# dtarb/TauDEM

Measured on NVIDIA H100. Metric: Mcells/s for aread8+areadinf on synthetic fractal DEM, higher is better.
Workload: dtype f32

## Files before the change

taudem_b200/csrc/sweep_warp.cu:

```cuda
#include <stddef.h>
#include <string.h>

#include <algorithm>

#include "ctx.h"
#include "dinf_common.cuh"
#include "kernels.h"
#include "rowfact.cuh"

namespace td {
namespace {

constexpr int TS = 32;
constexpr int TH = 32;
constexpr int RS = TS + 4;
constexpr int RH = TH + 2;
constexpr int RN = RH * RS + 4;
#ifndef TD_WSTK
#define TD_WSTK 128
#endif
constexpr int STKCAP = TD_WSTK;
constexpr unsigned NODE_VALID = 0x8000u, NODE_CON = 0x1000u;
constexpr unsigned FULL = 0xffffffffu;
constexpr int EXP_NO_CARRY = 16;
#ifdef TD_EMU
constexpr int MAXSH = 8;
#else
constexpr int MAXSH = 64;
#endif
constexpr int C_TERM = 3 * MAXSH * 16, C_ACTIVE = (3 * MAXSH + 1) * 16, C_WORDS = (3 * MAXSH + 2) * 16;

constexpr unsigned pack_dir(bool row) {
  unsigned v = 0;
  for (int k = 1; k <= 8; ++k) v |= (unsigned)((row ? drow(k) : dcol(k)) + 1) << (2 * k);
  return v;
}
constexpr unsigned DROW_LUT = pack_dir(true), DCOL_LUT = pack_dir(false);
__device__ __forceinline__ int lut_drow(int k) { return (int)((DROW_LUT >> (2 * k)) & 3u) - 1; }
__device__ __forceinline__ int lut_dcol(int k) { return (int)((DCOL_LUT >> (2 * k)) & 3u) - 1; }

template <bool DINF>
struct __align__(16) WarpMem {
  float area[RN];
  float ang[DINF ? RN : 4];
  unsigned short node[RN];
  alignas(16) unsigned cnt[TS * TH / 4];
  unsigned short stk[DINF ? STKCAP : 2];
  unsigned short ext[DINF ? 256 : 128];
  unsigned evmask[TH];
  int sp, next, ovf, pad;
};
template <bool DINF> constexpr int workers_per_cta() { return DINF ? 16 : 26; }
static_assert(sizeof(WarpMem<false>) * workers_per_cta<false>() <= 227 * 1024 && sizeof(WarpMem<true>) * workers_per_cta<true>() + 1024 <= 227 * 1024,
              "the workers of a CTA must fit the shared memory of an SM");
static_assert(offsetof(WarpMem<true>, ang) % 16 == 0 && offsetof(WarpMem<true>, node) % 8 == 0 && offsetof(WarpMem<false>, node) % 8 == 0, "cp.async alignment");

struct PeerStrip {
  unsigned* cntw = nullptr; int* state = nullptr; int* tq = nullptr; unsigned long long* ctr = nullptr; float* halo_in = nullptr;
  unsigned qmask = 0; int ntx = 0, ny = 0, valid = 0, nsh = 1, qshift = 0;
};

struct WArgs {
  const unsigned short* node;
  unsigned* cntw;
  float* area;
  const float* w;
  const float* ang;
  Strip s;
  int usew, contcheck;
  float w_nodata;
  const double* theta;
  const double* dxc;
  int* halo;
  int ntx, nty, th;
  const float* dm; float dm_nodata;
  const float* dist;
  SweepExtra x;
  int* state;
  int* tq;
  unsigned qmask;
  int nsh, qshift;
  PropRow prop;
  double dx0;
  unsigned long long* ctr;
  unsigned long long* stat;
  int stats, exp;
  int peer;
  PeerStrip up, down;
  unsigned long long* G;
  const float* halo_in;
};

#ifdef TD_EMU
template <typename T> __device__ __forceinline__ T ldv(const T* p) { emu::yield(); return *((const volatile T*)p); }
#else
template <typename T> __device__ __forceinline__ T ldv(const T* p) { return *((const volatile T*)p); }
#endif
template <typename T> __device__ __forceinline__ void stv(T* p, T v) { *((volatile T*)p) = v; }

#ifndef TD_EMU
__device__ __forceinline__ void cp16(void* smem, const void* g) { asm volatile("cp.async.cg.shared.global [%0], [%1], 16;" ::"r"(smem_u32(smem)), "l"(g) : "memory"); }
__device__ __forceinline__ void cp8(void* smem, const void* g) { asm volatile("cp.async.ca.shared.global [%0], [%1], 8;" ::"r"(smem_u32(smem)), "l"(g) : "memory"); }
__device__ __forceinline__ void cp4(void* smem, const void* g) { asm volatile("cp.async.ca.shared.global [%0], [%1], 4;" ::"r"(smem_u32(smem)), "l"(g) : "memory"); }
__device__ __forceinline__ void cp_wait_all() { asm volatile("cp.async.wait_all;" ::: "memory"); }
#else
__device__ __forceinline__ void cp_check(const void* smem, const void* g, size_t n) { if ((size_t)smem % n || (size_t)g % n) { fprintf(stderr, "emu: misaligned %zu-byte cp.async\n", n); abort(); } }
__device__ __forceinline__ void cp16(void* smem, const void* g) { emu::yield(); cp_check(smem, g, 16); memcpy(smem, g, 16); }
__device__ __forceinline__ void cp8(void* smem, const void* g) { cp_check(smem, g, 8); memcpy(smem, g, 8); }
__device__ __forceinline__ void cp4(void* smem, const void* g) { cp_check(smem, g, 4); memcpy(smem, g, 4); }
__device__ __forceinline__ void cp_wait_all() {}
#endif

#define W_ADD(ptr, v) (a.peer ? atomicAdd_system((ptr), (v)) : atomicAdd((ptr), (v)))
#define W_CAS(ptr, c, v) (a.peer ? atomicCAS_system((ptr), (c), (v)) : atomicCAS((ptr), (c), (v)))
#define W_EXCH(ptr, v) (a.peer ? atomicExch_system((ptr), (v)) : atomicExch((ptr), (v)))
#define W_ADD_IF(sys, ptr, v) ((sys) ? atomicAdd_system((ptr), (v)) : atomicAdd((ptr), (v)))
#define W_CAS_IF(sys, ptr, c, v) ((sys) ? atomicCAS_system((ptr), (c), (v)) : atomicCAS((ptr), (c), (v)))
#define W_EXCH_IF(sys, ptr, v) ((sys) ? atomicExch_system((ptr), (v)) : atomicExch((ptr), (v)))

__device__ __forceinline__ unsigned long long* w_head(unsigned long long* ctr, int q) { return ctr + (3 * q) * 16; }
__device__ __forceinline__ unsigned long long* w_tail(unsigned long long* ctr, int q) { return ctr + (3 * q + 1) * 16; }
__device__ __forceinline__ unsigned long long* w_done(unsigned long long* ctr, int q) { return ctr + (3 * q + 2) * 16; }

__device__ void sched_push(const WArgs& a, int t) {
  const int q = t & (a.nsh - 1);
  const unsigned long long slot = W_ADD(w_tail(a.ctr, q), 1ull);
  int* ring = a.tq + ((size_t)q << a.qshift) + (slot & a.qmask);
  while (W_CAS(ring, 0, t + 1) != 0) {}
}
__device__ __forceinline__ bool edge_tile(const WArgs& a, int t) { return a.peer && (t < a.ntx || t >= (a.nty - 1) * a.ntx); }
__device__ void sched_activate(const WArgs& a, int t) {
  const bool sys = edge_tile(a, t);
  for (;;) {
    const int st = W_CAS_IF(sys, a.state + t, 0, 1);
    if (st == 0) { sched_push(a, t); return; }
    if (st == 1 || st == 3) return;
    if (W_CAS_IF(sys, a.state + t, 2, 3) == 2) return;
  }
}
__device__ void sched_activate_peer(const WArgs& a, const PeerStrip& P, int t) {
  for (;;) {
    const int st = atomicCAS_system(P.state + t, 0, 1);
    if (st == 0) {
      atomicAdd_system(a.G, 1ull);
      const int q = t & (P.nsh - 1);
      const unsigned long long slot = atomicAdd_system(w_tail(P.ctr, q), 1ull);
      int* ring = P.tq + ((size_t)q << P.qshift) + (slot & P.qmask);
      while (atomicCAS_system(ring, 0, t + 1) != 0) {}
      __threadfence_system();
      if (atomicExch_system(P.ctr + C_ACTIVE, 1ull) == 1ull) atomicAdd_system(a.G, ~0ull);
      return;
    }
    if (st == 1 || st == 3) return;
    if (atomicCAS_system(P.state + t, 2, 3) == 2) return;
  }
}
template <int ALG>
__device__ void deliver_peer(const WArgs& a, bool up, int c_src, float val, int c_dst) {
  const PeerStrip& P = up ? a.up : a.down;
  const int pitch = a.s.pitch;
  P.halo_in[(up ? pitch : 0) + c_src] = val;
  if (ALG == 9) P.halo_in[2 * pitch + (up ? pitch : 0) + c_src] = ldv(a.x.out3 + a.s.idx(up ? 1 : a.s.ny, c_src));
  __threadfence_system();
  const int r = up ? P.ny : 1;
  const long long ci = (long long)r * pitch + c_dst;
  const unsigned sh = (unsigned)(ci & 3) * 8u;
  const unsigned old = atomicAdd_system(P.cntw + (ci >> 2), 0u - (1u << sh));
  if (((old >> sh) & 0xffu) == 1u) sched_activate_peer(a, P, ((r - 1) / a.th) * P.ntx + c_dst / TS);
}
__device__ __forceinline__ int ld_relaxed(const int* p) {
#ifdef TD_EMU
  emu::yield(); return *((const volatile int*)p);
#else
  int v; asm volatile("ld.relaxed.gpu.global.s32 %0, [%1];" : "=r"(v) : "l"(p) : "memory"); return v;
#endif
}
__device__ __forceinline__ long long ld_relaxed(const unsigned long long* p) {
#ifdef TD_EMU
  emu::yield(); return (long long)*((const volatile unsigned long long*)p);
#else
  long long v; asm volatile("ld.relaxed.gpu.global.s64 %0, [%1];" : "=l"(v) : "l"(p) : "memory"); return v;
#endif
}
__device__ __forceinline__ void idle_wait(unsigned cycles) {
#ifdef TD_EMU
  (void)cycles; emu::yield();
#else
  const long long t0 = clock64();
  do { __nanosleep(cycles >> 1); } while (clock64() - t0 < (long long)cycles);
#endif
}
__device__ __forceinline__ void fence_acquire(bool sys) {
#ifdef TD_EMU
  (void)sys; emu::yield();
#else
  if (sys) asm volatile("fence.acquire.sys;" ::: "memory");
  else asm volatile("fence.acquire.gpu;" ::: "memory");
#endif
}
__device__ __forceinline__ void fence_release(bool sys) {
#ifdef TD_EMU
  (void)sys; emu::yield();
#else
  if (sys) asm volatile("fence.release.sys;" ::: "memory");
  else asm volatile("fence.release.gpu;" ::: "memory");
#endif
}
__device__ __forceinline__ uint4 ld_cnt4(const uint4* p, bool sys) {
#ifdef TD_EMU
  (void)sys; return __ldcg(p);
#else
  uint4 v;
  if (sys) asm volatile("ld.relaxed.sys.global.v4.u32 {%0,%1,%2,%3}, [%4];" : "=r"(v.x), "=r"(v.y), "=r"(v.z), "=r"(v.w) : "l"(p) : "memory");
  else asm volatile("ld.relaxed.gpu.global.v4.u32 {%0,%1,%2,%3}, [%4];" : "=r"(v.x), "=r"(v.y), "=r"(v.z), "=r"(v.w) : "l"(p) : "memory");
  return v;
#endif
}
__device__ bool sched_balanced(const WArgs& a) {
  long long d = 0, t = 0;
#pragma unroll 16
  for (int q = 0; q < a.nsh; ++q) d += ld_relaxed(w_done(a.ctr, q));
  fence_acquire(false);
#pragma unroll 16
  for (int q = 0; q < a.nsh; ++q) t += ld_relaxed(w_tail(a.ctr, q));
  return d == t;
}
__device__ int sched_pop(const WArgs& a, int q, bool scanner) {
  const unsigned long long h = atomicAdd(w_head(a.ctr, q), 1ull);
  int* slot = a.tq + ((size_t)q << a.qshift) + (h & a.qmask);
  unsigned wait = 512, n = 0;
  for (;;) {
    const int v = ld_relaxed(slot);
    if (v != 0) {
      W_EXCH(slot, 0);
      const int prev = W_EXCH_IF(edge_tile(a, v - 1), a.state + (v - 1), 2);
      return prev == 0x7ffffff0 ? -1 : v - 1;
    }
    if ((++n & 7u) == 0u) {
      if (ld_relaxed(a.ctr + C_TERM) != 0) return -1;
      if (scanner && (n & 63u) == 0u && sched_balanced(a)) {
        bool over = true;
        if (a.peer) {
          if (atomicExch_system(a.ctr + C_ACTIVE, 0ull) == 1ull) {
            __threadfence_system();
            if (sched_balanced(a)) atomicAdd_system(a.G, ~0ull);
            else if (atomicExch_system(a.ctr + C_ACTIVE, 1ull) == 1ull) atomicAdd_system(a.G, ~0ull);
          }
          over = ldv(a.G) == 0ull;
        }
        if (over) { atomicExch(a.ctr + C_TERM, 1ull); return -1; }
      }
    }
    idle_wait(wait);
    if (wait < 4096) wait <<= 1;
  }
}
__device__ __forceinline__ int sched_release(const WArgs& a, int t, bool dirty) {
  return dirty ? 3 : W_CAS_IF(edge_tile(a, t), a.state + t, 2, 0);
}
__device__ void sched_finish(const WArgs& a, int t, int rel, bool pay) {
  if (rel != 2) { W_EXCH_IF(edge_tile(a, t), a.state + t, 1); sched_push(a, t); }
  if (pay) atomicAdd(w_done(a.ctr, t & (a.nsh - 1)), 1ull);
}

__global__ void k_zero_words(unsigned* p, size_t n) {
  for (size_t i = (size_t)blockIdx.x * blockDim.x + threadIdx.x; i < n; i += (size_t)gridDim.x * blockDim.x) p[i] = 0u;
}
__global__ void k_fill_floats(float* p, size_t n, float v) {
  for (size_t i = (size_t)blockIdx.x * blockDim.x + threadIdx.x; i < n; i += (size_t)gridDim.x * blockDim.x) p[i] = v;
}
unsigned fill_grid(size_t n) {
  int dev = 0, sms = 0;
  if (cudaGetDevice(&dev) != cudaSuccess || cudaDeviceGetAttribute(&sms, cudaDevAttrMultiProcessorCount, dev) != cudaSuccess || sms < 1) sms = 1;
  return (unsigned)std::max<size_t>(1, std::min<size_t>((n + 255) / 256, (size_t)sms * 16));
}
}
cudaError_t fill_floats(float* p, const Strip& s, float v, cudaStream_t st) {
  const size_t n = (size_t)s.cells();
  const unsigned grid = fill_grid(n);
  k_fill_floats<<<grid, 256, 0, st>>>(p, n, v);
  TD_LAUNCHED();
  return cudaGetLastError();
}
cudaError_t zero_words(void* p, size_t bytes, cudaStream_t st) {
  const size_t n = bytes / 4;
  const unsigned grid = fill_grid(n);
  k_zero_words<<<grid, 256, 0, st>>>((unsigned*)p, n);
  TD_LAUNCHED();
  return cudaGetLastError();
}
namespace {
__global__ void k_wsched_init(int* state, int* tq, int ntiles, unsigned long long* ctr, unsigned long long* stat, int nsh, int qshift, unsigned qmask) {
  const unsigned i = blockIdx.x * blockDim.x + threadIdx.x;
  if ((int)i < ntiles) {
    state[i] = 1;
    const int q = (int)i & (nsh - 1);
    const unsigned long long slot = atomicAdd(w_tail(ctr, q), 1ull);
    tq[((size_t)q << qshift) + (slot & qmask)] = (int)i + 1;
  }
  if (i == 0) {
    ctr[C_ACTIVE] = 1ull;
    for (int j = 0; j < 9; ++j) stat[j] = 0;
  }
}

__device__ __noinline__ double wshare_full(float ang, double t, int kk) {
  const Outflow o = dinf_outflow(ang, t);
  return o.k1 == kk ? o.p1 : o.p2;
}
struct __align__(16) Sector { double lo, hi, den, rden; };

__device__ __forceinline__ unsigned zero_bytes(unsigned w) { return ~(((w & 0x7f7f7f7fu) + 0x7f7f7f7fu) | w) & 0x80808080u; }
__device__ __forceinline__ unsigned zero_nibble(unsigned w) {
  const unsigned z = zero_bytes(w);
  return ((z >> 7) & 1u) | ((z >> 14) & 2u) | ((z >> 21) & 4u) | ((z >> 28) & 8u);
}

template <int ALG, typename Mem>
__device__ __forceinline__ float gridnet_eval(const WArgs& a, const Mem& M, int ri, unsigned msk, int r, int c) {
  const Strip& s = a.s;
  if (a.dm && a.dm[s.idx(r, c)] == 0.f) return a.w_nodata;
  const float* drowp = a.dist + (size_t)(min(r, s.ny) - 1) * 8;
  float val = 0.f, a1 = 0.f, a2 = 0.f;
#pragma unroll
  for (int k = 1; k <= 8; ++k) {
    if (!(msk & (1u << (k - 1)))) continue;
    const int ni = ri + drow(k) * RS + dcol(k);
    if ((((unsigned)M.node[ni] >> 8) & 0xfu) == 0u) continue;
    if (a.dm && a.dm[s.idx(r + drow(k), c + dcol(k))] == 0.f) continue;
    const float an = M.area[ni];
    const float d = drowp[k - 1];
    if (ALG == 4) { const float ld = an + d; if (ld > val) val = ld; }
    else if (ALG == 5) val = val + (an + d);
    else { if (an >= a1) { a2 = a1; a1 = an; } else if (an > a2) a2 = an; }
  }
  if (ALG == 6) val = (a2 + 1.f > a1) ? a2 + 1.f : a1;
  return val;
}

struct Eval { float val; bool con; };
template <bool USEW, int ALG, typename Mem>
__device__ __forceinline__ Eval d8_gather(const WArgs& a, const Mem& M, int ri, unsigned msk, int r, int c, float wv, float NOD, bool con) {
  if (ALG >= 4) return {gridnet_eval<ALG>(a, M, ri, msk, r, c), con};
  if (USEW) {
    float val = (ALG == 0 && nd_f(wv, a.w_nodata)) ? -1.0f : wv;
#pragma unroll
    for (int k = 1; k <= 8; ++k)
      if (msk & (1u << (k - 1))) {
        const float an = M.area[ri + drow(k) * RS + dcol(k)];
        if (nd_f(an, NOD)) con = true;
        else val = ALG == 0 ? val + an : ALG == 1 ? (an > val ? an : val) : (an < val ? an : val);
      }
    return {val, con};
  }
  float val = 1.0f, mn = 0.f;
#pragma unroll
  for (int k = 1; k <= 8; ++k)
    if (msk & (1u << (k - 1))) {
      const float an = M.area[ri + drow(k) * RS + dcol(k)];
      val = val + an;
      mn = fminf(mn, an);
    }
  if (mn < 0.f) con = true;
  return {val, con};
}

__device__ __forceinline__ double dinf_share(const WArgs& a, const Sector* sect, unsigned f, float av, int kk, int rn) {
  if (a.prop.uniform && f != 9u) {
    const bool upper = f >= 10u;
    const int k1 = (int)(upper ? f - 8u : f);
    const bool first = kk == k1 && !upper;
    const bool wrap = k1 == 8 && !first && !upper;
    const Sector S = sect[wrap ? 0 : (upper ? k1 - 1 : k1)];
    double ad = (double)av;
    if (wrap) ad = (double)(float)(ad - 2.0 * TD_PI);
    const double num = first ? S.hi - ad : ad - S.lo;
    return a.prop.safe ? div_recip(num, S.den, S.rden) : num / S.den;
  }
  return wshare_full(av, a.prop.uniform ? a.prop.ar[2] : theta_of_row(a.theta, a.s.ny, min(max(rn, 0), a.s.ny + 1)), kk);
}

__device__ __forceinline__ double own_area(const WArgs& a, int r) { return a.prop.uniform ? a.dx0 : a.dxc[min(r, a.s.ny) - 1]; }

template <bool DINF, bool USEW, int ALG>
__global__ void __launch_bounds__(workers_per_cta<DINF>() * 32, 1) k_sweep_warp(const WArgs a) {
  extern __shared__ __align__(16) unsigned char dsm[];
  using Mem = WarpMem<DINF>;
  const Strip& s = a.s;
  const int lane = (int)(threadIdx.x & 31u), wid = (int)(threadIdx.x >> 5);
  const unsigned lt = (1u << lane) - 1u;
  Mem& M = *reinterpret_cast<Mem*>(dsm + (size_t)wid * sizeof(Mem));
  const int myq = (int)((blockIdx.x * (blockDim.x >> 5) + (unsigned)wid) & (unsigned)(a.nsh - 1));
  const float NOD = (ALG == 0 || (ALG >= 4 && ALG <= 6)) ? -1.0f : TD_MISSINGFLOAT;
  __shared__ Sector sect[9];
  if (DINF) {
    if (threadIdx.x < 9) { const int j = (int)threadIdx.x; sect[j].lo = a.prop.ar[j]; sect[j].hi = a.prop.ar[j + 1]; sect[j].den = a.prop.den[j]; sect[j].rden = a.prop.rden[j]; }
    __syncthreads();
  }

  int carry = -1;
  for (;;) {
    long long tk0 = 0, tk1 = 0, tk2 = 0, tk3 = 0;
    int t = carry;
    if (t < 0) {
      if (lane == 0) { if (a.stats) tk0 = clock64(); t = sched_pop(a, myq, wid == 0); if (a.stats) tk1 = clock64(); }
      t = __shfl_sync(FULL, t, 0);
      if (t < 0) return;
    } else if (a.stats && lane == 0) { tk0 = clock64(); tk1 = tk0; }
    carry = -1;
    const int ty = t / a.ntx, tx = t - ty * a.ntx;
    const int c0 = tx * TS, r0 = 1 + ty * TH;

    unsigned g0[8];
    {
      const int r = r0 + lane;
      uint4 qa = make_uint4(FULL, FULL, FULL, FULL), qb = qa;
      if (r <= s.ny) {
        const uint4* src = reinterpret_cast<const uint4*>(a.cntw + (s.idx(r, c0) >> 2));
        qa = ld_cnt4(src, a.peer); qb = ld_cnt4(src + 1, a.peer);
      }
      g0[0] = qa.x; g0[1] = qa.y; g0[2] = qa.z; g0[3] = qa.w; g0[4] = qb.x; g0[5] = qb.y; g0[6] = qb.z; g0[7] = qb.w;
      uint4* dst = reinterpret_cast<uint4*>(M.cnt + lane * 8);
      dst[0] = qa; dst[1] = qb;
      M.evmask[lane] = 0u;
    }
    if (lane == 0) { M.sp = 0; M.next = 0; M.ovf = 0; }
    fence_acquire(a.peer);
    __syncwarp();
#pragma unroll
    for (int j = 0; j < (RH * 8 + 31) / 32; ++j) {
      const int i = lane + 32 * j;
      if (i < RH * 8) {
        const int rr = i >> 3, q = i & 7;
        const int r = r0 - 1 + rr, c = c0 + 4 * q;
        const int so = rr * RS + 4 + 4 * q;
        if (r <= s.ny + 1) {
          const long long g = s.idx(r, c);
          if (a.peer && (r == 0 || r == s.ny + 1)) cp16(M.area + so, a.halo_in + (r == 0 ? 0 : s.pitch) + c);
          else cp16(M.area + so, a.area + g);
          if (DINF) cp16(M.ang + so, a.ang + g);
          cp8(M.node + so, a.node + g);
        } else {
          *reinterpret_cast<float4*>(M.area + so) = make_float4(NOD, NOD, NOD, NOD);
          if (DINF) *reinterpret_cast<float4*>(M.ang + so) = make_float4(0.f, 0.f, 0.f, 0.f);
          *reinterpret_cast<uint2*>(M.node + so) = make_uint2(0u, 0u);
        }
      }
    }
#pragma unroll
    for (int rr = lane; rr < RH; rr += 32) {
      const int r = r0 - 1 + rr;
      const bool rowok = r <= s.ny + 1;
      const bool halo_row = a.peer && (r == 0 || r == s.ny + 1);
      const float* hrow = a.halo_in + (r == 0 ? 0 : s.pitch);
      const int sw = rr * RS + 3, se = rr * RS + RS;
      const bool west = rowok && c0 > 0, east = rowok && c0 + TS < s.pitch;
      const long long gw_ = s.idx(r, c0 - 1), ge_ = s.idx(r, c0 + TS);
      float aw = NOD, ae = NOD;
      if (west) { aw = __ldcg(halo_row ? hrow + (c0 - 1) : a.area + gw_); if (DINF) cp4(M.ang + sw, a.ang + gw_); cp4(M.node + sw - 1, a.node + gw_ - 1); }
      else { M.node[sw - 1] = 0; M.node[sw] = 0; }
      if (east) { ae = __ldcg(halo_row ? hrow + (c0 + TS) : a.area + ge_); if (DINF) cp4(M.ang + se, a.ang + ge_); cp4(M.node + se, a.node + ge_); }
      else { M.node[se] = 0; M.node[se + 1] = 0; }
      M.area[sw] = aw; M.area[se] = ae;
    }
    unsigned rdy = 0;
#pragma unroll
    for (int j = 0; j < 8; ++j) rdy |= zero_nibble(g0[j]) << (4 * j);
    cp_wait_all();
    __syncwarp();
    if (a.stats && lane == 0) tk2 = clock64();

    int cur = -1;
    int iters = 0;
    for (;;) {
      if (cur < 0 && rdy) { const int b = __ffs(rdy) - 1; rdy &= rdy - 1; cur = lane * TS + b; }
      if (DINF) {
        const unsigned idle = __ballot_sync(FULL, cur < 0);
        if (idle) {
          const int n = min(ldv(&M.sp), STKCAP);
          if (n > 0) {
            const int take = min(__popc(idle), n);
            const int rank = __popc(idle & lt);
            if (cur < 0 && rank < take) cur = M.stk[n - 1 - rank];
            __syncwarp();
            if (lane == 0) M.sp = n - take;
          }
        }
      }
      const unsigned act = __ballot_sync(FULL, cur >= 0);
      if (ALG < 7 && act != 0u && (act & (act - 1u)) == 0u) {
        int c = __shfl_sync(FULL, cur, __ffs(act) - 1);
        bool forked = false;
        do {
          ++iters;
          const int lr = c >> 5, lx = c & 31;
          const int ri = (lr + 1) * RS + lx + 4;
          float wv = 0.f;
          if (USEW) wv = a.w[s.idx(r0 + lr, c0 + lx)];
          const unsigned nd = M.node[ri];
          const unsigned msk = nd & 0xffu;
          bool con = (nd & NODE_CON) != 0;
          float val;
          if (!DINF) { const Eval e = d8_gather<USEW, ALG>(a, M, ri, msk, r0 + lr, c0 + lx, wv, NOD, con); val = e.val; con = e.con; }
          else {
            double prod = 0.;
            if (lane < 8 && ((msk >> lane) & 1u)) {
              const int k = lane + 1;
              const int dr = lut_drow(k);
              const int ni = ri + dr * RS + lut_dcol(k);
              const unsigned f = ((unsigned)M.node[ni] >> 8) & 0xfu;
              const float av = M.ang[ni];
              const float an = M.area[ni];
              const double p = dinf_share(a, sect, f, av, k > 4 ? k - 4 : k + 4, r0 + lr + dr);
              if (ALG == 3) {
                const float dmv = __ldg(a.dm + s.idx(r0 + lr + dr, c0 + lx + lut_dcol(k)));
                prod = (nd_f(an, NOD) || nd_f(dmv, a.dm_nodata)) ? __longlong_as_double(0x7ff8dead00000000ll) : (double)(float)((double)(dmv * an) * p);
              } else prod = nd_f(an, NOD) ? __longlong_as_double(0x7ff8dead00000000ll) : p * (double)an;
            }
            val = 0.f;
            if (ALG == 3) val = USEW ? wv : (float)own_area(a, r0 + lr);
            for (unsigned m = msk; m; m &= m - 1u) {
              const double pr = __shfl_sync(FULL, prod, __ffs(m) - 1);
              if (pr != pr) con = true; else val = ALG == 3 ? val + (float)pr : (float)((double)val + pr);
            }
            if (ALG == 3) {}
            else if (USEW) val = val + wv;
            else val = (float)((double)val + own_area(a, r0 + lr));
          }
          if (con && a.contcheck) val = NOD;
          if (lane == 0) { M.area[ri] = val; M.evmask[lr] |= 1u << lx; }
          int next = -1;
#pragma unroll
          for (int j = 0; j < (DINF ? 2 : 1); ++j) {
            int k;
            if (!DINF) k = (int)((nd >> 8) & 0xfu);
            else k = j == 0 ? dinf_node_k1(nd) : dinf_node_k2(nd);
            if (k < 1 || k > 8) continue;
            const int nlr = lr + lut_drow(k), nlx = lx + lut_dcol(k);
            if ((unsigned)nlr < (unsigned)TH && (unsigned)nlx < (unsigned)TS && r0 + nlr <= s.ny) {
              const int l2 = nlr * TS + nlx;
              const unsigned sh = (unsigned)(l2 & 3) * 8u;
              unsigned w = 0;
              if (lane == 0) { w = M.cnt[l2 >> 2]; M.cnt[l2 >> 2] = w - (1u << sh); }
              w = __shfl_sync(FULL, w, 0);
              if (((w >> sh) & 0xffu) == 1u) {
                if (next < 0) next = l2;
                else {
                  forked = true;
                  if (lane == 0) { const int slot = M.sp; if (slot < STKCAP) M.stk[slot] = (unsigned short)l2; else if (a.stats) M.ovf = 1; M.sp = slot + 1; }
                }
              }
            } else if (s.on_grid(r0 + nlr, c0 + nlx)) {
              if (lane == 0) { M.ext[M.next] = (unsigned short)(c | ((k - 1) << 11)); M.next = M.next + 1; }
            }
          }
          c = next;
          __syncwarp();
        } while (c >= 0 && !forked);
        cur = lane == 0 ? c : -1;
        continue;
      }
      if (act == 0u) {
        if (!DINF) break;
        const unsigned ev = M.evmask[lane];
#pragma unroll
        for (int j = 0; j < 8; ++j) rdy |= zero_nibble(M.cnt[lane * 8 + j]) << (4 * j);
        rdy &= ~ev;
        if (__ballot_sync(FULL, rdy != 0u) == 0u) break;
        continue;
      }
      ++iters;
      if (cur >= 0) {
        const int l = cur;
        const int lr = l >> 5, lx = l & 31;
        const int ri = (lr + 1) * RS + lx + 4;
        float wv = 0.f;
        if (USEW) wv = a.w[s.idx(r0 + lr, c0 + lx)];
        const unsigned nd = M.node[ri];
        const unsigned msk = nd & 0xffu;
        bool con = (nd & NODE_CON) != 0;
        float val;
        int cont = -1;
        if (!DINF) { const Eval e = d8_gather<USEW, ALG>(a, M, ri, msk, r0 + lr, c0 + lx, wv, NOD, con); val = e.val; con = e.con; }
        else {
          const int r = r0 + lr;
          val = 0.f;
          float loadin = 0.f;
          if (ALG == 3) val = USEW ? wv : (float)own_area(a, r);
#pragma unroll 1
          for (unsigned m = msk; m; m &= m - 1u) {
            const int k = __ffs(m);
            const int dr = lut_drow(k);
            const int ni = ri + dr * RS + lut_dcol(k);
            const unsigned f = ((unsigned)M.node[ni] >> 8) & 0xfu;
            const float av = M.ang[ni];
            const float an = M.area[ni];
            const double p = dinf_share(a, sect, f, av, k > 4 ? k - 4 : k + 4, r + dr);
            if (ALG == 3) {
              const float dmv = __ldg(a.dm + s.idx(r + dr, c0 + lx + lut_dcol(k)));
              if (nd_f(an, NOD) || nd_f(dmv, a.dm_nodata)) con = true;
              else val = val + (float)((double)(dmv * an) * p);
            } else if (ALG == 7) {
              const long long gi = s.idx(r + dr, c0 + lx + lut_dcol(k));
              const float qq = __ldg(a.w + gi), dmm = __ldg(a.dm + gi);
              if (nd_f(an, NOD) || nd_f(dmm, a.dm_nodata) || nd_f(qq, a.w_nodata)) con = true;
              else val = (float)((double)val + ((p * (double)an) * (double)qq) * (double)dmm);
            } else if (ALG == 8 || ALG == 9) {
              float nt = 0.f;
              if (nd_f(an, NOD)) con = true; else { val = (float)((double)val + p * (double)an); nt = an; }
              if (ALG == 9) {
                const int rn = r + dr, cc = c0 + lx + lut_dcol(k);
                const float cn = (a.peer && (rn == 0 || rn == s.ny + 1)) ? ldv(a.halo_in + 2 * s.pitch + (rn == 0 ? 0 : s.pitch) + cc)
                                                                         : ldv(a.x.out3 + s.idx(rn, cc));
                if (nd_f(cn, NOD)) con = true; else loadin = (float)((double)loadin + (p * (double)nt) * (double)cn);
              }
            } else if (nd_f(an, NOD)) con = true; else val = (float)((double)val + p * (double)an);
          }
          if (ALG == 3) {}
          else if (ALG == 7) {
            const float dgv = (float)a.x.dg[s.idx(r, c0 + lx)];
            if (!(wv > 0.f)) { val = NOD; con = false; }
            else if (dgv > 0.f) { val = a.x.csol; con = false; }
            else val = val / wv;
          } else if (ALG == 8 || ALG == 9) {
            const long long gc = s.idx(r, c0 + lx);
            const float tcc = __ldg(a.dm + gc);
            float cinv = 0.f;
            bool ev = !nd_f(wv, a.w_nodata) && !nd_f(tcc, a.dm_nodata);
            if (ALG == 9) { cinv = __ldg(a.x.cin + gc); ev = ev && !nd_f(cinv, a.x.cin_nodata); }
            if (!ev) { val = NOD; con = false; }
            else {
              const float transin = val;
              float transout, depp;
              if ((transin + wv) > tcc) { transout = tcc; depp = transin + wv - transout; }
              else { transout = transin + wv; depp = 0.f; }
              float cs = 0.f;
              if (ALG == 9) {
                float loadout;
                if (transout < transin) loadout = transin > 0.f ? loadin * transout / transin : 0.f;
                else loadout = loadin + cinv * (transout - transin);
                cs = transout > 0.f ? loadout / transout : 0.f;
              }
              const bool bad = con && a.contcheck;
              a.x.out2[gc] = bad ? NOD : depp;
              if (ALG == 9) { stv(a.x.out3 + gc, bad ? NOD : cs); __threadfence_block(); }
              val = transout;
            }
          }
          else if (USEW) val = val + wv;
          else val = (float)((double)val + own_area(a, r));
        }
        if (con && a.contcheck) val = NOD;
        M.area[ri] = val;
        atomicOr(&M.evmask[lr], 1u << lx);
#pragma unroll
        for (int j = 0; j < (DINF ? 2 : 1); ++j) {
          int k;
          if (!DINF) k = (int)((nd >> 8) & 0xfu);
          else k = j == 0 ? dinf_node_k1(nd) : dinf_node_k2(nd);
          if (k < 1 || k > 8) continue;
          const int nlr = lr + lut_drow(k), nlx = lx + lut_dcol(k);
          if ((unsigned)nlr < (unsigned)TH && (unsigned)nlx < (unsigned)TS && r0 + nlr <= s.ny) {
            const int l2 = nlr * TS + nlx;
            const unsigned sh = (unsigned)(l2 & 3) * 8u;
            const unsigned old = atomicSub(&M.cnt[l2 >> 2], 1u << sh);
            if (((old >> sh) & 0xffu) == 1u) {
              if (cont < 0) cont = l2;
              else {
                const int slot = atomicAdd(&M.sp, 1);
                if (slot < STKCAP) M.stk[slot] = (unsigned short)l2; else if (a.stats) M.ovf = 1;
              }
            }
          } else if (s.on_grid(r0 + nlr, c0 + nlx)) {
            M.ext[atomicAdd(&M.next, 1)] = (unsigned short)(l | ((k - 1) << 11));
          }
        }
        cur = cont;
      }
      __syncwarp();
    }

    if (a.stats && lane == 0) tk3 = clock64();

    const unsigned evs = M.evmask[lane];
    for (unsigned rows = __ballot_sync(FULL, evs != 0u); rows; rows &= rows - 1u) {
      const int lr = __ffs(rows) - 1;
      const unsigned evr = __shfl_sync(FULL, evs, lr);
      if ((evr >> lane) & 1u) a.area[s.idx(r0 + lr, c0 + lane)] = M.area[(lr + 1) * RS + lane + 4];
    }
    unsigned dl[8];
    {
      const int myr = r0 + lane;
      const bool rimrow = lane == 0 || lane == TH - 1 || myr >= s.ny;
      unsigned* gw = a.cntw + (s.idx(min(myr, s.ny), c0) >> 2);
#pragma unroll
      for (int j = 0; j < 8; ++j) {
        const unsigned was = g0[j];
        unsigned now = M.cnt[lane * 8 + j];
        const unsigned keep = ((was >> 7) & 0x01010101u) * 0xffu;
        now = (now & ~keep) | (was & keep);
        const unsigned e4 = (evs >> (4 * j)) & 0xfu;
        dl[j] = now - was + ((e4 * 0x00204081u) & 0x01010101u) * 0xfeu;
        if (j >= 1 && j <= 6 && !rimrow && dl[j] != 0u) { gw[j] = was + dl[j]; dl[j] = 0u; }
      }
    }
    __syncwarp();
    fence_release(a.peer);
    const int ne = M.next;
    int pend = -1, pend_e = -1;
    auto cross = [&](int e, unsigned& old, unsigned& sh) -> int {
      const int l = M.ext[e] & 0x7ff, k = (M.ext[e] >> 11) + 1;
      const int lr = l >> 5, lx = l & 31;
      const int nlr = lr + lut_drow(k), nlx = lx + lut_dcol(k);
      const int r = r0 + nlr, c = c0 + nlx;
      if (r == 0 || r == s.ny + 1) {
        if (a.peer) deliver_peer<ALG>(a, r == 0, c0 + lx, M.area[(lr + 1) * RS + lx + 4], c);
        else atomicAdd(a.halo + (r == 0 ? 0 : s.pitch) + c, 1);
        return -1;
      }
      if (!((unsigned)M.node[(nlr + 1) * RS + nlx + 4] & NODE_VALID)) return -1;
      const long long ci = s.idx(r, c);
      sh = (unsigned)(ci & 3) * 8u;
      old = W_ADD_IF(a.peer && (r == 1 || r == s.ny), a.cntw + (ci >> 2), 0u - (1u << sh));
      return ((r - 1) / TH) * a.ntx + c / TS;
    };
    unsigned xo = 0u, xsh = 0u, ro[8];
    const int xt = lane < ne ? cross(lane, xo, xsh) : -1;
    const int myr = r0 + lane;
#pragma unroll
    for (int j = 0; j < 8; ++j) ro[j] = 0u;
    if (myr <= s.ny) {
      unsigned* gw = a.cntw + (s.idx(myr, c0) >> 2);
#pragma unroll
      for (int j = 0; j < 8; ++j)
        if (dl[j] != 0u) ro[j] = W_ADD_IF(a.peer && (myr == 1 || myr == s.ny), gw + j, dl[j]);
    }
    if (xt >= 0 && ((xo >> xsh) & 0xffu) == 1u) { pend = xt; pend_e = lane; }
    for (int e = lane + 32; e < ne; e += 32) {
      unsigned o, sh;
      const int tt = cross(e, o, sh);
      if (tt >= 0 && ((o >> sh) & 0xffu) == 1u) {
        if (pend >= 0) sched_activate(a, pend);
        pend = tt; pend_e = e;
      }
    }
    bool dirty = false;
#pragma unroll
    for (int j = 0; j < 8; ++j)
      if (dl[j] != 0u && zero_bytes(ro[j] + dl[j])) dirty = true;
    dirty = __ballot_sync(FULL, dirty) != 0u;
    int hi = pend_e;
#pragma unroll
    for (int d = 16; d >= 1; d >>= 1) hi = max(hi, __shfl_xor_sync(FULL, hi, d));
    const int wl = hi & 31;
    const int ct = hi >= 0 ? __shfl_sync(FULL, pend, wl) : -1;
    int claim = -1, rel = -1;
    if (hi >= 0 && lane == wl && !(a.exp & EXP_NO_CARRY)) claim = W_CAS_IF(edge_tile(a, ct), a.state + ct, 0, 2);
    if (lane == 0) rel = sched_release(a, t, dirty);
    if (hi >= 0) {
      if (lane == wl) {
        if (claim == 0) {
          carry = ct;
          if (a.stats) atomicAdd(a.stat, 1ull);
        } else sched_activate(a, ct);
      } else if (pend >= 0 && pend != ct) sched_activate(a, pend);
      carry = __shfl_sync(FULL, carry, wl);
    }
    __syncwarp();
    if (lane == 0) sched_finish(a, t, rel, carry < 0);
    if (a.stats) {
      int tot = __popc(evs);
#pragma unroll
      for (int d = 16; d >= 1; d >>= 1) tot += __shfl_xor_sync(FULL, tot, d);
      if (lane == 0) {
        const long long tk4 = clock64();
        atomicAdd(a.stat + 3, 1ull);
        atomicAdd(a.stat + 4, (unsigned long long)(tk1 - tk0));
        atomicAdd(a.stat + 5, (unsigned long long)(tk2 - tk1));
        atomicAdd(a.stat + 6, (unsigned long long)(tk3 - tk2));
        atomicAdd(a.stat + 7, (unsigned long long)(tk4 - tk3));
        atomicAdd(a.stat + 1, (unsigned long long)tot);
        atomicAdd(a.stat + 2, (unsigned long long)iters);
        if (DINF && M.ovf) atomicAdd(a.stat + 8, 1ull);
      }
    }
    __syncwarp();
  }
}

__global__ void k_wapply_halo(WArgs a, const int* __restrict__ dec_top, const int* __restrict__ dec_bot) {
  const int c = blockIdx.x * blockDim.x + threadIdx.x;
  if (c >= a.s.nx) return;
#pragma unroll
  for (int side = 0; side < 2; ++side) {
    const int* dec = side == 0 ? dec_top : dec_bot;
    if (dec == nullptr) continue;
    const int d = dec[c];
    if (d <= 0) continue;
    const int r = side == 0 ? 1 : a.s.ny;
    const long long ci = a.s.idx(r, c);
    if (!(a.node[ci] & NODE_VALID)) continue;
    const unsigned sh = (unsigned)(ci & 3) * 8u;
    const unsigned old = atomicAdd(a.cntw + (ci >> 2), 0u - ((unsigned)d << sh));
    if ((int)((old >> sh) & 0xffu) == d) sched_activate(a, ((r - 1) / a.th) * a.ntx + c / TS);
  }
}

__global__ void k_wsched_reset(unsigned long long* ctr) { for (int i = threadIdx.x; i < C_WORDS; i += blockDim.x) ctr[i] = (i == C_ACTIVE) ? 1ull : 0ull; }

int wargs(td_ctx* ctx, WArgs& a, const Strip& s) {
  a.s = s;
  a.area = nullptr; a.w = nullptr; a.ang = nullptr; a.dx0 = 0.; a.usew = 0; a.contcheck = 1; a.w_nodata = 0.f; a.theta = nullptr; a.dxc = nullptr; a.halo = nullptr; a.dm = nullptr; a.dm_nodata = 0.f; a.dist = nullptr;
  a.th = TH;
  a.ntx = (s.nx + TS - 1) / TS; a.nty = (s.ny + a.th - 1) / a.th;
  a.stats = 0; a.exp = 0;
  a.peer = 0; a.G = nullptr; a.halo_in = nullptr; a.up = PeerStrip(); a.down = PeerStrip();
  const long long nt = (long long)a.ntx * a.nty;
  if (nt > (1ll << 30)) { set_error("strip has too many tiles"); return TD_ERR_ARG; }
  int nsh = 1;
  while (nsh * 2 <= MAXSH && nsh * 2 <= nt) nsh *= 2;
  const unsigned long long need = (unsigned long long)((nt + nsh - 1) / nsh) + (1u << 13);
  int qshift = 14;
  while ((1ull << qshift) < need) ++qshift;
  a.nsh = nsh; a.qshift = qshift; a.qmask = (1u << qshift) - 1u;
  TD_CUDA(ctx->tileflags.ensure((size_t)nt * 4 + ((size_t)nsh << qshift) * 4));
  a.state = ctx->tileflags.as<int>();
  a.tq = a.state + nt;
  TD_CUDA(ctx->wsched.ensure(C_WORDS * sizeof(unsigned long long)));
  a.ctr = ctx->wsched.as<unsigned long long>();
  a.stat = ctx->d_ctr + 24;
  a.node = ctx->node.as<unsigned short>();
  a.cntw = ctx->cnt.as<unsigned>();
  return TD_OK;
}

enum : unsigned { NEED_W = 1, NEED_DM = 2, NEED_DIST = 4, NEED_EXTRA = 8, NEED_DG = 16, NEED_OUT2 = 32, NEED_CIN = 64, NEED_OUT3 = 128 };
using SweepLaunch = void (*)(const WArgs&, int, int, size_t, cudaStream_t);
template <bool D, bool U, int A>
void launch_sweep(const WArgs& a, int g, int threads, size_t smem, cudaStream_t st) {
  k_sweep_warp<D, U, A><<<g, threads, smem, st>>>(a);
}
struct SweepKernel {
  bool dinf, usew;
  int alg;
  unsigned need;
  const void* kern;
  SweepLaunch launch;
  int threads;
  size_t smem;
};
template <bool D, bool U, int A>
SweepKernel sweep_kernel(unsigned need) {
  return {D, U, A, need, (const void*)k_sweep_warp<D, U, A>, launch_sweep<D, U, A>, workers_per_cta<D>() * 32, sizeof(WarpMem<D>) * workers_per_cta<D>()};
}
const SweepKernel SWEEPS[] = {
    sweep_kernel<false, false, 0>(0), sweep_kernel<false, true, 0>(0), sweep_kernel<true, false, 0>(0), sweep_kernel<true, true, 0>(0),
    sweep_kernel<false, true, 1>(0), sweep_kernel<false, true, 2>(0),
    sweep_kernel<true, false, 3>(NEED_DM), sweep_kernel<true, true, 3>(NEED_DM),
    sweep_kernel<false, false, 4>(NEED_DIST), sweep_kernel<false, false, 5>(NEED_DIST), sweep_kernel<false, false, 6>(NEED_DIST),
    sweep_kernel<true, true, 7>(NEED_W | NEED_DM | NEED_EXTRA | NEED_DG),
    sweep_kernel<true, true, 8>(NEED_W | NEED_DM | NEED_EXTRA | NEED_OUT2),
    sweep_kernel<true, true, 9>(NEED_W | NEED_DM | NEED_EXTRA | NEED_OUT2 | NEED_CIN | NEED_OUT3),
};
static_assert(sizeof(SWEEPS) / sizeof(SWEEPS[0]) == td_ctx::SWEEP_KERNELS, "td_ctx::wgrid has one slot per sweep kernel");
}

int wsweep_begin(td_ctx* ctx, const Strip& s, cudaStream_t st) {
  WArgs a;
  if (int rc = wargs(ctx, a, s)) return rc;
  const int nt = a.ntx * a.nty;
  TD_CUDA(zero_words(a.ctr, C_WORDS * sizeof(unsigned long long), st));
  TD_CUDA(zero_words(a.tq, ((size_t)a.nsh << a.qshift) * sizeof(int), st));
  k_wsched_init<<<(nt + 255) / 256, 256, 0, st>>>(a.state, a.tq, nt, a.ctr, a.stat, a.nsh, a.qshift, a.qmask);
  TD_LAUNCHED();
  TD_CUDA(cudaGetLastError());
  return TD_OK;
}

int wsweep_apply_halo(td_ctx* ctx, const Strip& s, const int* dec_top, const int* dec_bot, cudaStream_t st) {
  WArgs a;
  if (int rc = wargs(ctx, a, s)) return rc;
  k_wsched_reset<<<1, 256, 0, st>>>(a.ctr);
  TD_LAUNCHED();
  k_wapply_halo<<<(s.nx + 255) / 256, 256, 0, st>>>(a, dec_top, dec_bot);
  TD_LAUNCHED();
  TD_CUDA(cudaGetLastError());
  return TD_OK;
}

int wsweep_run(td_ctx* ctx, bool dinf, float* area, const float* w, const float* ang, const Strip& s, float w_nodata, int usew,
               int contcheck, const double* theta, const double* dxc, int* halo, cudaStream_t st, int alg, const float* dm, float dm_nodata,
               const float* dist, const SweepExtra* extra) {
  int row = -1;
  for (int i = 0; i < td_ctx::SWEEP_KERNELS; ++i)
    if (SWEEPS[i].dinf == dinf && SWEEPS[i].usew == (usew != 0) && SWEEPS[i].alg == alg) row = i;
  const unsigned have = (w ? NEED_W : 0u) | (dm ? NEED_DM : 0u) | (dist ? NEED_DIST : 0u) |
                        (extra ? NEED_EXTRA | (extra->dg ? NEED_DG : 0u) | (extra->out2 ? NEED_OUT2 : 0u) | (extra->cin ? NEED_CIN : 0u) | (extra->out3 ? NEED_OUT3 : 0u) : 0u);
  if (row < 0) { set_error("wsweep_run: no sweep for this algebra with this flow model and weights"); return TD_ERR_ARG; }
  if (const unsigned miss = SWEEPS[row].need & ~have) {
    static const char* const grid[8] = {"w", "dm", "dist", "extra", "extra->dg", "extra->out2", "extra->cin", "extra->out3"};
    set_error(std::string("wsweep_run: algebra ") + std::to_string(alg) + " requires the grid " + grid[__builtin_ctz(miss)]);
    return TD_ERR_ARG;
  }
  const SweepKernel& K = SWEEPS[row];
  if (alg == 9 && ctx->peer_on && ctx->peer_halo.cap < sizeof(float) * 4 * (size_t)s.pitch) {
    set_error("wsweep_run: peer mode of the transport limited accumulation with a concentration needs the halo buffer of sweep_peer_export");
    return TD_ERR_ARG;
  }
  WArgs a;
  if (int rc = wargs(ctx, a, s)) return rc;
  a.area = area; a.w = w; a.ang = ang; a.usew = usew; a.contcheck = contcheck;
  a.w_nodata = w_nodata; a.theta = theta; a.dxc = dxc; a.halo = halo; a.dm = dm; a.dm_nodata = dm_nodata; a.dist = dist;
  if (extra) a.x = *extra;
  a.prop = ctx->prop;
  if (!dinf) a.prop.uniform = 0;
  a.peer = ctx->peer_on;
  if (a.peer) {
    auto fill = [](const td_ctx::PeerInfo& pi, PeerStrip& P) {
      P.valid = pi.valid;
      P.cntw = (unsigned*)pi.cntw; P.state = (int*)pi.tileflags; P.tq = P.state + pi.nt; P.ctr = (unsigned long long*)pi.dctr;
      P.halo_in = (float*)pi.halo_in; P.qmask = (unsigned)pi.qmask; P.ntx = pi.ntx; P.ny = pi.ny; P.nsh = pi.nsh; P.qshift = pi.qshift;
    };
    fill(ctx->peer_up, a.up); fill(ctx->peer_down, a.down);
    a.G = (unsigned long long*)ctx->peer_G;
    a.halo_in = ctx->peer_halo.as<float>();
    if ((s.has_top && !a.up.valid) || (s.has_bot && !a.down.valid) || !a.G) { set_error("peer mode: neighbours are not connected"); return TD_ERR_ARG; }
  }
  const char* te = getenv("TAUDEM_B200_TIMING");
  a.stats = (te && atoi(te) > 0) ? 1 : 0;
  if (const char* xe = getenv("TAUDEM_B200_EXP")) a.exp = atoi(xe);
  a.dx0 = ctx->dx0;
  int& per_dev = ctx->wgrid[row];
  if (!per_dev) {
    int dev = 0, sms = 0, occ = 0;
    TD_CUDA(cudaGetDevice(&dev));
    TD_CUDA(cudaDeviceGetAttribute(&sms, cudaDevAttrMultiProcessorCount, dev));
    TD_CUDA(cudaFuncSetAttribute(K.kern, cudaFuncAttributeMaxDynamicSharedMemorySize, (int)K.smem));
    TD_CUDA(cudaOccupancyMaxActiveBlocksPerMultiprocessor(&occ, K.kern, K.threads, K.smem));
    if (occ < 1) { set_error("sweep kernel does not fit on an SM"); return TD_ERR_CUDA; }
    per_dev = sms * occ;
  }
  const long long nt = (long long)a.ntx * a.nty;
  const int warps = K.threads / 32;
  K.launch(a, (int)std::min<long long>(per_dev, (nt + warps - 1) / warps), K.threads, K.smem, st);
  TD_LAUNCHED();
  TD_CUDA(cudaGetLastError());
  return TD_OK;
}

namespace {
__global__ void k_add_G(unsigned long long* G, unsigned long long v) { if (threadIdx.x == 0) { atomicAdd_system(G, v); __threadfence_system(); } }
void close_peer(td_ctx::PeerInfo& pi) {
  if (pi.cntw) cudaIpcCloseMemHandle(pi.cntw);
  if (pi.tileflags) cudaIpcCloseMemHandle(pi.tileflags);
  if (pi.dctr) cudaIpcCloseMemHandle(pi.dctr);
  if (pi.halo_in) cudaIpcCloseMemHandle(pi.halo_in);
  pi = td_ctx::PeerInfo();
}
}

int sweep_peer_export(td_ctx* ctx, const Strip& s, int dinf, unsigned char* handles, int* meta, cudaStream_t st) {
  WArgs a;
  ctx->sweep_dinf = dinf ? 1 : 0;
  const size_t n = (size_t)s.cells();
  TD_CUDA(ctx->node.ensure(n * 2));
  TD_CUDA(ctx->cnt.ensure((n + 3) / 4 * 4));
  if (int rc = wargs(ctx, a, s)) return rc;
  TD_CUDA(ctx->peer_halo.ensure(sizeof(float) * 4 * (size_t)s.pitch));
  TD_CUDA(ctx->gbuf.ensure(64));
  TD_CUDA(cudaMemsetAsync(ctx->gbuf.p, 0, 64, st));
  TD_CUDA(cudaStreamSynchronize(st));
  void* ptrs[5] = {ctx->cnt.p, ctx->tileflags.p, ctx->wsched.p, ctx->peer_halo.p, ctx->gbuf.p};
  for (int i = 0; i < 5; ++i) {
    cudaIpcMemHandle_t h;
    TD_CUDA(cudaIpcGetMemHandle(&h, ptrs[i]));
    memcpy(handles + 64 * i, &h, 64);
  }
  meta[0] = (int)a.qmask; meta[1] = a.ntx; meta[2] = s.ny; meta[3] = a.th; meta[4] = a.ntx * a.nty; meta[5] = a.nsh; meta[6] = a.qshift; meta[7] = 0;
  return TD_OK;
}

int sweep_peer_connect(td_ctx* ctx, int which, const unsigned char* handles, const int* meta) {
  auto open = [](const unsigned char* h64, void** out) -> cudaError_t {
    cudaIpcMemHandle_t h; memcpy(&h, h64, 64);
    return cudaIpcOpenMemHandle(out, h, cudaIpcMemLazyEnablePeerAccess);
  };
  if (which == 2) {
    if (ctx->peer_G_opened && ctx->peer_G) cudaIpcCloseMemHandle(ctx->peer_G);
    ctx->peer_G_opened = false;
    if (!handles) { ctx->peer_G = ctx->gbuf.p; return TD_OK; }
    TD_CUDA(open(handles + 64 * 4, &ctx->peer_G));
    ctx->peer_G_opened = true;
    return TD_OK;
  }
  td_ctx::PeerInfo& pi = which == 0 ? ctx->peer_up : ctx->peer_down;
  if (!handles && meta && pi.valid) {
    pi.qmask = meta[0]; pi.ntx = meta[1]; pi.ny = meta[2]; pi.th = meta[3]; pi.nt = meta[4]; pi.nsh = meta[5]; pi.qshift = meta[6];
    return TD_OK;
  }
  close_peer(pi);
  if (!handles) return TD_OK;
  TD_CUDA(open(handles, &pi.cntw));
  TD_CUDA(open(handles + 64, &pi.tileflags));
  TD_CUDA(open(handles + 128, &pi.dctr));
  TD_CUDA(open(handles + 192, &pi.halo_in));
  pi.qmask = meta[0]; pi.ntx = meta[1]; pi.ny = meta[2]; pi.th = meta[3]; pi.nt = meta[4]; pi.nsh = meta[5]; pi.qshift = meta[6]; pi.valid = 1;
  return TD_OK;
}

int sweep_peer_begin(td_ctx* ctx, const Strip& s, cudaStream_t st) {
  ctx->peer_on = 1;
  if (int rc = wsweep_begin(ctx, s, st)) return rc;
  WArgs a;
  if (int rc = wargs(ctx, a, s)) return rc;
  TD_CUDA(zero_words(ctx->peer_halo.p, sizeof(float) * 4 * (size_t)s.pitch, st));
  k_add_G<<<1, 32, 0, st>>>((unsigned long long*)ctx->peer_G, 1ull);
  TD_LAUNCHED();
  TD_CUDA(cudaStreamSynchronize(st));
  return TD_OK;
}
void sweep_peer_off(td_ctx* ctx) { ctx->peer_on = 0; }

}
```

Measured before the change: 2560.

## Batch single-active D8 chains into warp-wide runs with shuffle prefix accumulation

When only one cell is ready in a tile for D8 area (ALG 0), lane 0 now walks the downstream chain serially, collecting up to 32 cells whose other inflows are already resolved. All lanes then gather the off-chain contributions in parallel, and the chain values are accumulated with a shuffle-up scan. This is meant to replace one warp iteration per chain cell with one iteration per run. In exchange it adds a serial walk on lane 0, a quadratic-looking shuffle loop, extra shared memory for the run buffer, and new stats counters.

```diff
diff --git a/taudem_b200/csrc/sweep_warp.cu b/taudem_b200/csrc/sweep_warp.cu
--- a/taudem_b200/csrc/sweep_warp.cu
+++ b/taudem_b200/csrc/sweep_warp.cu
@@ -48,7 +48,8 @@
   unsigned short stk[DINF ? STKCAP : 2];
   unsigned short ext[DINF ? 256 : 128];
   unsigned evmask[TH];
-  int sp, next, ovf, pad;
+  unsigned short run[DINF ? 2 : TS];
+  int sp, next, ovf, runs;
 };
 template <bool DINF> constexpr int workers_per_cta() { return DINF ? 16 : 26; }
 static_assert(sizeof(WarpMem<false>) * workers_per_cta<false>() <= 227 * 1024 && sizeof(WarpMem<true>) * workers_per_cta<true>() + 1024 <= 227 * 1024,
@@ -300,7 +301,7 @@
   }
   if (i == 0) {
     ctr[C_ACTIVE] = 1ull;
-    for (int j = 0; j < 9; ++j) stat[j] = 0;
+    for (int j = 0; j < 11; ++j) stat[j] = 0;
   }
 }
 
@@ -381,6 +382,95 @@
 }
 
 __device__ __forceinline__ double own_area(const WArgs& a, int r) { return a.prop.uniform ? a.dx0 : a.dxc[min(r, a.s.ny) - 1]; }
+
+constexpr int RUN_POST = 3;
+template <bool USEW>
+__device__ __forceinline__ int chain_run(const WArgs& a, WarpMem<false>& M, int c, int r0, int c0, int lane) {
+  const Strip& s = a.s;
+  const float NOD = -1.0f;
+  int n = 0, nxt = -1;
+  if (lane == 0) {
+    int x = c, kin = 0;
+    unsigned nd = M.node[(x >> 5) * RS + RS + (x & 31) + 4];
+    for (;;) {
+      const int lr = x >> 5, lx = x & 31;
+      if (n > 0 && __popc((nd & 0xffu) >> kin) > RUN_POST) break;
+      M.run[n++] = (unsigned short)(x | (kin << 11));
+      nxt = -1;
+      const int k = (int)((nd >> 8) & 0xfu);
+      if (k >= 1 && k <= 8) {
+        const int nlr = lr + lut_drow(k), nlx = lx + lut_dcol(k);
+        if ((unsigned)nlr < (unsigned)TH && (unsigned)nlx < (unsigned)TS && r0 + nlr <= s.ny) {
+          const int l2 = nlr * TS + nlx;
+          const unsigned sh = (unsigned)(l2 & 3) * 8u;
+          const unsigned w = M.cnt[l2 >> 2];
+          const unsigned ndl = M.node[(nlr + 1) * RS + nlx + 4];
+          M.cnt[l2 >> 2] = w - (1u << sh);
+          if (((w >> sh) & 0xffu) == 1u) { nxt = l2; nd = ndl; kin = k > 4 ? k - 4 : k + 4; }
+        } else if (s.on_grid(r0 + nlr, c0 + nlx)) {
+          M.ext[M.next] = (unsigned short)(x | ((k - 1) << 11)); M.next = M.next + 1;
+        }
+      }
+      if (nxt < 0 || n == TS) break;
+      x = nxt;
+    }
+    if (a.stats) M.runs += n | (1 << 16);
+  }
+  __syncwarp();
+  n = __shfl_sync(FULL, n, 0); nxt = __shfl_sync(FULL, nxt, 0);
+
+  int ri = 0, kin = 0, lr = 0, lx = 0, np = 0;
+  float val = 0.f, post[RUN_POST];
+  bool con = false;
+#pragma unroll
+  for (int q = 0; q < RUN_POST; ++q) post[q] = 0.f;
+  if (lane < n) {
+    const unsigned e = M.run[lane];
+    kin = (int)(e >> 11);
+    lr = (int)(e >> 5) & 31; lx = (int)e & 31;
+    ri = (lr + 1) * RS + lx + 4;
+    const float wv = USEW ? a.w[s.idx(r0 + lr, c0 + lx)] : 0.f;
+    const unsigned nd = M.node[ri];
+    const unsigned msk = nd & 0xffu;
+    con = (nd & NODE_CON) != 0;
+    const int kc = kin ? kin : 9;
+    float mn = 0.f;
+    val = !USEW ? 1.0f : nd_f(wv, a.w_nodata) ? -1.0f : wv;
+#pragma unroll
+    for (int k = 1; k <= 8; ++k) {
+      if (!((msk >> (k - 1)) & 1u) || k == kin) continue;
+      const float an = M.area[ri + drow(k) * RS + dcol(k)];
+      if (USEW && nd_f(an, NOD)) { con = true; continue; }
+      mn = fminf(mn, an);
+      if (k < kc) val = val + an;
+      else {
+#pragma unroll
+        for (int q = 0; q + 1 < RUN_POST; ++q) post[q] = post[q + 1];
+        post[RUN_POST - 1] = an; ++np;
+      }
+    }
+    if (!USEW && mn < 0.f) con = true;
+  }
+
+  float res = 0.f;
+  for (int j = 0; j < n; ++j) {
+    const float up = __shfl_up_sync(FULL, res, 1);
+    float v = val;
+    bool cn = con;
+    if (kin) {
+      if (USEW) { if (nd_f(up, NOD)) cn = true; else v = v + up; }
+      else { v = v + up; if (up < 0.f) cn = true; }
+    }
+#pragma unroll
+    for (int q = 0; q < RUN_POST; ++q)
+      if (q >= RUN_POST - np) v = v + post[q];
+    if (cn && a.contcheck) v = NOD;
+    if (lane == j) res = v;
+  }
+  if (lane < n) { M.area[ri] = res; atomicOr(&M.evmask[lr], 1u << lx); }
+  __syncwarp();
+  return nxt;
+}
 
 template <bool DINF, bool USEW, int ALG>
 __global__ void __launch_bounds__(workers_per_cta<DINF>() * 32, 1) k_sweep_warp(const WArgs a) {
@@ -424,7 +514,7 @@
       dst[0] = qa; dst[1] = qb;
       M.evmask[lane] = 0u;
     }
-    if (lane == 0) { M.sp = 0; M.next = 0; M.ovf = 0; }
+    if (lane == 0) { M.sp = 0; M.next = 0; M.ovf = 0; M.runs = 0; }
     fence_acquire(a.peer);
     __syncwarp();
 #pragma unroll
@@ -491,7 +581,12 @@
       if (ALG < 7 && act != 0u && (act & (act - 1u)) == 0u) {
         int c = __shfl_sync(FULL, cur, __ffs(act) - 1);
         bool forked = false;
-        do {
+        if constexpr (ALG == 0 && !DINF) {
+          do {
+            ++iters;
+            c = chain_run<USEW>(a, M, c, r0, c0, lane);
+          } while (c >= 0);
+        } else do {
           ++iters;
           const int lr = c >> 5, lx = c & 31;
           const int ri = (lr + 1) * RS + lx + 4;
@@ -782,6 +877,7 @@
         atomicAdd(a.stat + 1, (unsigned long long)tot);
         atomicAdd(a.stat + 2, (unsigned long long)iters);
         if (DINF && M.ovf) atomicAdd(a.stat + 8, 1ull);
+        if (const unsigned ru = (unsigned)M.runs) { atomicAdd(a.stat + 9, (unsigned long long)(ru & 0xffffu)); atomicAdd(a.stat + 10, (unsigned long long)(ru >> 16)); }
       }
     }
     __syncwarp();
```

Result: no change. 2574 (median of 6 runs) (+0.6%).
